# getreu/stringsext

Measured on AMD Instinct MI355X. Metric: GiB/s scanned, higher is better.
Workload: dtype u8

## Files before the change

### stringsext_amd/csrc/sx_api.cpp

```cpp
#include "sx_ctx.hpp"

using namespace sx;

namespace sx {
PinnedPool::Block PinnedPool::take(size_t bytes) {
    {
        std::lock_guard<std::mutex> g(mu);
        size_t best = free_blocks.size();
        for (size_t i = 0; i < free_blocks.size(); i++)
            if (free_blocks[i].cap >= bytes && (best == free_blocks.size() || free_blocks[i].cap < free_blocks[best].cap)) best = i;
        if (best < free_blocks.size() && free_blocks[best].cap <= 4 * bytes + (4u << 20)) {
            Block b = free_blocks[best];
            free_blocks.erase(free_blocks.begin() + (long)best);
            return b;
        }
    }
    Block b;
    const size_t cap = bytes + bytes / 8 + (1u << 20);
    if (hipHostMalloc(&b.p, cap, hipHostMallocNonCoherent) != hipSuccess) { b.p = nullptr; return b; }
    b.cap = cap;
    return b;
}
void PinnedPool::give(Block b) {
    if (!b.p) return;
// ... 254 lines not shown
                         + ", requested=" + std::to_string(hip_device) + "); the scan only runs on the GPU";
        delete ctx;
        return SX_E_NO_DEVICE;
    }
    ctx->device = hip_device;
    auto fail = [&](const char* what, hipError_t err) {
        g_create_error = std::string(what) + ": " + hipGetErrorString(err);
        sx_destroy(ctx);
        return SX_E_HIP;
    };
    if ((e = hipSetDevice(hip_device)) != hipSuccess) return fail("hipSetDevice", e);
    ctx->dev.resize((size_t)n_missions);
    const uint32_t cap = ctx->opt.record_capacity ? ctx->opt.record_capacity : (1u << 20);
    {
        int cus = 0;
        if (hipDeviceGetAttribute(&cus, hipDeviceAttributeMultiprocessorCount, hip_device) == hipSuccess && cus > 0) ctx->n_cus = (unsigned)cus;
        if (ctx->sw.scan_blocks_per_cu >= 0) ctx->scan_blocks_per_cu = (unsigned)ctx->sw.scan_blocks_per_cu;
        if (ctx->sw.region_cap >= 0) ctx->region_cap = (uint32_t)ctx->sw.region_cap;
        if (ctx->sw.scan_cus) ctx->n_cus = (unsigned)ctx->sw.scan_cus;
    }
    int prio_lo = 0, prio_hi = 0;
    (void)hipDeviceGetStreamPriorityRange(&prio_lo, &prio_hi);
    if (ctx->sw.prio_n >= 0) {
        if (ctx->sw.prio_n >= 1) prio_lo = ctx->sw.prio_scan;
        if (ctx->sw.prio_n >= 2) prio_hi = ctx->sw.prio_post;
        fprintf(stderr, "[sx] stream priorities: scan %d, post %d\n", prio_lo, prio_hi);
    }
    const bool per_mission = (ctx->opt.flags & SX_OPT_MISSION_STREAMS) || ctx->sw.mission_streams;
    if ((e = hipStreamCreateWithPriority(&ctx->post_stream, hipStreamNonBlocking, prio_hi)) != hipSuccess) return fail("hipStreamCreate", e);
    if (!per_mission && (e = hipStreamCreateWithPriority(&ctx->scan_stream, hipStreamNonBlocking, prio_lo)) != hipSuccess)
        return fail("hipStreamCreate", e);
// ... 55 lines not shown
            if (d.h_runs) (void)hipHostFree(d.h_runs);
            if (d.ev_runs) (void)hipEventDestroy(d.ev_runs);
            if (d.stream_w) (void)hipStreamDestroy(d.stream_w);
            if (d.h_tot) (void)hipHostFree(d.h_tot);
            if (d.h_small) (void)hipHostFree(d.h_small);
            for (hipEvent_t e : d.wave_ev) if (e) (void)hipEventDestroy(e);
            if (d.stream && d.stream != ctx->scan_stream) (void)hipStreamDestroy(d.stream);
        }
        for (int i = 0; i < 2; i++) {
            if (ctx->ing_pin[i]) (void)hipHostFree(ctx->ing_pin[i]);
            if (ctx->ing_dev[i]) (void)hipFree(ctx->ing_dev[i]);
        }
        if (ctx->copy_stream) (void)hipStreamDestroy(ctx->copy_stream);
        if (ctx->d2h_stream) (void)hipStreamDestroy(ctx->d2h_stream);
        if (ctx->scan_stream) (void)hipStreamDestroy(ctx->scan_stream);
        if (ctx->d_cache) (void)hipFree(ctx->d_cache);
        if (ctx->post_stream) (void)hipStreamDestroy(ctx->post_stream);
        if (ctx->merge_copy_stream) (void)hipStreamDestroy(ctx->merge_copy_stream);
        if (ctx->d_merge) (void)hipFree(ctx->d_merge);
        if (ctx->d_result) (void)hipFree(ctx->d_result);
        if (ctx->d_result_up) (void)hipFree(ctx->d_result_up);
        if (ctx->d_text) (void)hipFree(ctx->d_text);
        if (ctx->d_print_scratch) (void)hipFree(ctx->d_print_scratch);
        if (ctx->d_print_missions) (void)hipFree(ctx->d_print_missions);
        for (uint8_t* p : ctx->d_select) if (p) (void)hipFree(p);
        if (ctx->d_select_scratch) (void)hipFree(ctx->d_select_scratch);
        if (ctx->d_select_scratch2) (void)hipFree(ctx->d_select_scratch2);
        if (ctx->d_distinct) (void)hipFree(ctx->d_distinct);
        for (hipEvent_t e : ctx->merge_ev) if (e) (void)hipEventDestroy(e);
        for (hipEvent_t e : ctx->slab_ev) if (e) (void)hipEventDestroy(e);
// ... 248 lines not shown
```

### stringsext_amd/csrc/sx_ctx.hpp

```cpp
#pragma once
#include <hip/hip_runtime_api.h>
#include <stdio.h>
#include <stdlib.h>
#include <string.h>
#include <errno.h>
#include <fcntl.h>
#include <sys/mman.h>
#include <sys/stat.h>
#include <unistd.h>

#include <algorithm>
#include <atomic>
#include <chrono>
#include <condition_variable>
#include <deque>
#include <functional>
#include <mutex>
#include <string>
#include <thread>
#include <unordered_map>
#include <vector>

#include "sx_host.hpp"
#include "sx_switches.hpp"
#include "sx_stage_b_plan.hpp"

namespace sx {

double now_ms();
constexpr size_t kSmallReadBytes = 4096;
extern double g_tl_t0;
extern int g_tl_on;
#define SX_TL(...) do { if (sx::g_tl_on) { fprintf(stderr, "[tl %+8.3f] ", sx::now_ms() - sx::g_tl_t0); fprintf(stderr, __VA_ARGS__); fputc('\n', stderr); } } while (0)

struct RunList {
    std::vector<sx_run> own;
    const sx_run* p = nullptr;
    size_t n = 0;
    bool on_device = false;
    bool skipped = false;
// ... 97 lines not shown

struct sx_ctx {
    std::shared_ptr<sx::PinnedPool> pool = std::make_shared<sx::PinnedPool>();
    std::shared_ptr<std::atomic<uint64_t>> dev_epoch = std::make_shared<std::atomic<uint64_t>>(0);
    std::vector<sx::Mission> missions;
    std::vector<sx::ScannerState> states;
    std::vector<sx::MissionDev> dev;
    bool host_only = false;
    bool sharded_call = false, single_piece = true;
    int device = -1;
    sx_options opt{};
    sx::Switches sw;
    std::string err;
    sx_stats stats{};
    hipStream_t scan_stream = nullptr, post_stream = nullptr;
    uint8_t* d_cache = nullptr;
    uint64_t d_cache_cap = 0;
    hipStream_t merge_copy_stream = nullptr;
    hipEvent_t merge_ev[3] = { nullptr, nullptr, nullptr };
    hipEvent_t slab_ev[3] = { nullptr, nullptr, nullptr };
    std::atomic<bool> slab_copy_pending{ false };
    uint8_t* d_merge = nullptr; uint64_t d_merge_cap = 0, merge_out_room = 0, merge_n_out = 0;
    uint8_t* d_result = nullptr; uint64_t d_result_cap = 0;
    uint8_t* d_result_up = nullptr; uint64_t d_result_up_cap = 0;
    uint8_t* d_text = nullptr; uint64_t d_text_cap = 0;
    uint8_t* d_print_scratch = nullptr; uint64_t d_print_scratch_cap = 0;
    uint8_t* d_print_missions = nullptr;
    uint8_t* d_select[2] = { nullptr, nullptr }; uint64_t d_select_cap[2] = { 0, 0 };
    std::shared_ptr<std::atomic<uint64_t>> select_epoch[2] = { std::make_shared<std::atomic<uint64_t>>(0), std::make_shared<std::atomic<uint64_t>>(0) };
    uint64_t select_calls = 0;
    uint8_t* d_select_scratch = nullptr; uint64_t d_select_scratch_cap = 0;
    uint8_t* d_select_scratch2 = nullptr; uint64_t d_select_scratch2_cap = 0;
    uint8_t* d_distinct = nullptr; uint64_t d_distinct_cap = 0;
    bool merge_async = false;
    bool merge_copy_pending[2] = { false, false };
    uint64_t merge_parts = 0;
    uint64_t merged_out_bytes = 0;
    double out_density = 0;
    hipEvent_t ev_interleaved = nullptr;
    std::atomic<bool> interleave_pending{ false };
    std::mutex mu;
    std::mutex err_mu;
    std::recursive_mutex grow_mu;
    void set_err(std::string text) { std::lock_guard<std::mutex> g(err_mu); err = std::move(text); }
    unsigned n_cus = 256, scan_blocks_per_cu = 8;
    hipStream_t copy_stream = nullptr;
    hipStream_t d2h_stream = nullptr;
    uint8_t* ing_pin[2] = { nullptr, nullptr };
    uint8_t* ing_dev[2] = { nullptr, nullptr };
    uint64_t ing_cap = 0, ing_dev_cap = 0;
    uint32_t region_cap = 64;
    std::vector<uint32_t> dense;
    uint8_t* d_input = nullptr;
    uint64_t d_input_cap = 0;
    uint64_t ondemand_fetches = 0;
    std::vector<uint64_t> last_runs;
    std::vector<char> wave_pred;
    std::vector<double> wave_density;
    std::vector<char> wave_off;
    std::vector<sx::RunList> shard_runs;
// ... 78 lines not shown
int read_back_sync(sx_ctx* ctx, sx::MissionDev& d, hipStream_t s, void* host_dst, const void* dev_src, size_t bytes);
int read_back_async(sx_ctx* ctx, hipStream_t s, void* pinned_dst, const void* dev_src, size_t bytes);
int ensure_scratch(sx_ctx* ctx, uint64_t bytes);
int ensure_capacity(sx_ctx* ctx, ScanSlot& s, uint32_t cap);
int ensure_rp(sx_ctx* ctx, MissionDev& d, int slot, uint64_t bytes);
int ensure_cache(sx_ctx* ctx, uint64_t bytes);
unsigned usable_cpus();
unsigned replay_threads(const sx_ctx* ctx);
void begin_call(sx_ctx* ctx);
void fill_segment_info(const MissionFindings& s, sx_segment_info* info);

ScanParams scan_params(const sx_ctx* ctx, int mission, const ScanSlot& s, const uint8_t* d_bytes, uint64_t len,
                       uint32_t parity, uint64_t min_chars);
int stage_a_launch(sx_ctx* ctx, const std::vector<int>& which, const uint8_t* d_bytes, uint64_t len,
                   const std::vector<uint32_t>& parity, const std::vector<uint64_t>& min_chars, int si);
struct ReplayJob;
int ensure_copy_stream(sx_ctx* ctx);
bool result_stays_on_device(const sx_ctx* ctx, const ReplayJob& job);
int merge_drain(sx_ctx* ctx);
int slab_copy_drain(sx_ctx* ctx);
int stage_a_finish(sx_ctx* ctx, const std::vector<int>& which, const uint8_t* d_bytes, uint64_t len,
                   const std::vector<uint32_t>& parity, const std::vector<uint64_t>& min_chars, int si,
                   std::vector<RunList>* out, bool cut_into_pieces = false, const ReplayJob* wave_job = nullptr);
int device_runs(sx_ctx* ctx, const std::vector<int>& which, const uint8_t* d_bytes, uint64_t len,
                const std::vector<uint32_t>& parity, const std::vector<uint64_t>& min_chars,
                std::vector<RunList>* out);

struct ReplayJob {
    uint64_t len = 0;
    int file_id = -1;
// ... 97 lines not shown
```

### stringsext_amd/csrc/sx_device.hpp

```cpp
#pragma once
#include <cstdlib>
#include <hip/hip_runtime_api.h>
#include <stdint.h>

#include "../../include/stringsext_amd.h"

namespace sx {

constexpr uint32_t kTileBytes = 1024;

struct DevRun {
    uint64_t start;
    uint32_t len;
    uint32_t chars_flags;
};
constexpr uint32_t kRecStartOpen = 0x80000000u;
constexpr uint32_t kRecEndOpen = 0x40000000u;
constexpr uint32_t kRecCharsMask = 0x3FFFFFFFu;
constexpr uint32_t kRecInvalidLen = 0xFFFFFFFFu, kRecInvalidFlags = 0xFFFFFFFFu;

constexpr uint32_t kStatBase = 32, kStatShards = 16, kStatStride = 32, kCounterWords = kStatBase + kStatShards * kStatStride;

enum ClassifierKind : uint32_t {
    kClsSingleByteLut = 0,
// ... 250 lines not shown
size_t merge_scratch_bytes(uint32_t n);
hipError_t merge_sorted_records(const DevRun* recs, uint32_t n, uint64_t min_chars, void* scratch, size_t scratch_bytes,
                                sx_run* out, uint32_t* out_count, hipStream_t stream);

hipError_t launch_scan(ClassifierKind kind, const ScanParams& p, hipStream_t stream);
constexpr int kFusedMax = 3;
struct FusedParams {
    ScanParams m[kFusedMax];
    const uint8_t* data;
    uint64_t len;
    uint32_t subchunk;
    uint32_t fsh[kFusedMax][4];
    uint32_t cand_f[kFusedMax];
    uint32_t pf_zero[kFusedMax];
};
int fused_slot_of(ClassifierKind kind, const ScanParams& p);
hipError_t launch_scan_fused(const FusedParams& fp, uint32_t used, hipStream_t stream, int prefilter_override);
hipError_t launch_fill_background(uint8_t* dst, uint64_t first_index, uint64_t len, uint64_t seed,
                                  hipStream_t stream);
hipError_t launch_read_sum(const uint8_t* src, uint64_t len, uint64_t* out, hipStream_t stream, uint32_t subchunk = 0, uint32_t rot = 0);
hipError_t launch_gather(const uint8_t* src, uint8_t* dst, const uint64_t* seg_src, const uint64_t* seg_dst,
                         const uint32_t* seg_len, uint32_t n, hipStream_t stream);

}
```

### stringsext_amd/csrc/sx_fused.hip

```cpp
#include "sx_scan_core.hpp"

namespace sx {

struct NoCls {};

SX_DEV u32 shr1_keep(u32 v, u32 old) { return __builtin_amdgcn_update_dpp(old, v, 0x138, 0xF, 0xF, false); }
SX_DEV u32 ror1(u32 v) { return __builtin_amdgcn_mov_dpp(v, 0x13C, 0xF, 0xF, false); }

static_assert(offsetof(FusedParams, m) == 0, "late_params addresses m[slot] from the start of the kernel-argument segment");
typedef const __attribute__((address_space(4))) ScanParams* KArgMission;
SX_DEV KArgMission late_params(u32 slot) {
    asm volatile("" : "+s"(slot));
    return (KArgMission)__builtin_amdgcn_kernarg_segment_ptr() + slot;
}

struct LateEmitter {
    u32 slot, wave;
    u32 rcount, heavy_n;
    SX_DEV void append(bool want, u64 start, u64 end, u32 chars, u32 flags) {
        const u64 m = __ballot(want);
        if (m == 0) return;
        const KArgMission mp = late_params(slot);
        const u32 cap = mp->region_cap;
        DevRun* const recs = mp->recs;
// ... 314 lines not shown
                    const u32 suf = trailing_ones16(S.c.g63 & 0xFFFFu);
                    const u32 s63 = starts_before(*cls, toff, after);
                    os = after - suf;
                    och = (u32)__popc((s63 & 0xFFFFu) >> (16u - suf));
                    ofl = 0;
                }
                S.em.append(lane == 0, os, sub_end, och, ofl | kRecEndOpen);
            }
            S.em.end_region();
        }
    };
    finish(s0); finish(s1); finish(s2);
}

template <class C0, class C1, class C2>
static hipError_t launch_f(const FusedParams& fp, uint32_t used, hipStream_t stream, int prefilter_override) {
    const u64 waves = (fp.len + fp.subchunk - 1) / fp.subchunk;
    const u64 blocks = (waves + 3) / 4;
    if (blocks == 0) return hipSuccess;
    FusedParams q = fp;
    int mode = 1;
    if ((used & 2u) && Prefilter<C1>::mode_for(fp.m[1]) != 1) mode = Prefilter<C1>::mode_for(fp.m[1]);
    if ((used & 4u) && mode && Prefilter<C2>::mode_for(fp.m[2]) != 1) mode = Prefilter<C2>::mode_for(fp.m[2]) == 0 ? 0 : 2;
    if (!(used & 6u)) mode = 0;
    if (prefilter_override == 0) mode = 0; else if (prefilter_override == 2 && mode == 1) mode = 2;
    q.pf_zero[0] = 0; q.pf_zero[1] = Prefilter<C1>::zero_bits(fp.m[1]); q.pf_zero[2] = Prefilter<C2>::zero_bits(fp.m[2]);
    if (mode == 1) hipLaunchKernelGGL((scan_kernel_fused<C0, C1, C2, 1>), dim3((unsigned)blocks), dim3(256), 0, stream, q);
    else if (mode == 2) hipLaunchKernelGGL((scan_kernel_fused<C0, C1, C2, 2>), dim3((unsigned)blocks), dim3(256), 0, stream, q);
    else hipLaunchKernelGGL((scan_kernel_fused<C0, C1, C2, 0>), dim3((unsigned)blocks), dim3(256), 0, stream, q);
    return hipGetLastError();
}

int fused_slot_of(ClassifierKind kind, const ScanParams& p) {
    if (p.region_cap == 0 || p.persistent) return -1;
    if (kind == kClsUtf8Range2) return 0;
    if (kind == kClsUtf16Range) return p.big_endian ? 2 : 1;
    return -1;
}

hipError_t launch_scan_fused(const FusedParams& fp, uint32_t used, hipStream_t stream, int prefilter_override) {
    u32 parity = 0;
    if (used & 2u) parity = fp.m[1].parity & 1u; else if (used & 4u) parity = fp.m[2].parity & 1u;
    FusedParams q = fp;
    for (int s = 0; s < kFusedMax; s++) {
        if (!((used >> s) & 1u)) continue;
        q.data = fp.m[s].data; q.len = fp.m[s].len; q.subchunk = fp.m[s].subchunk;
        const u32 c = std::min<u32>(fp.m[s].cand_bytes, 12u);
        q.cand_f[s] = c;
        u32 have = 1;
        const u32 sh0 = have < c ? 1u : 0u; have += sh0;
        const u32 sh1 = have < c ? std::min(have, c - have) : 0u; have += sh1;
        const u32 rem = c - have;
        const u32 sh2 = std::min(have, rem), sh3 = rem;
        q.fsh[s][0] = sh0; q.fsh[s][1] = sh1; q.fsh[s][2] = sh2; q.fsh[s][3] = sh3;
    }
#define SX_ARG(...) __VA_ARGS__
#define SX_F(U, P, A, B, C) if (used == U && parity == P) return launch_f<A, B, C>(q, used, stream, prefilter_override);
    SX_F(1u, 0u, Utf8Range2, NoCls, NoCls)
    SX_F(7u, 0u, Utf8Range2, SX_ARG(Utf16RangeT<0, 0>), SX_ARG(Utf16RangeT<1, 0>))
    SX_F(7u, 1u, Utf8Range2, SX_ARG(Utf16RangeT<0, 1>), SX_ARG(Utf16RangeT<1, 1>))
    SX_F(3u, 0u, Utf8Range2, SX_ARG(Utf16RangeT<0, 0>), NoCls)
    SX_F(3u, 1u, Utf8Range2, SX_ARG(Utf16RangeT<0, 1>), NoCls)
    SX_F(5u, 0u, Utf8Range2, NoCls, SX_ARG(Utf16RangeT<1, 0>))
    SX_F(5u, 1u, Utf8Range2, NoCls, SX_ARG(Utf16RangeT<1, 1>))
    SX_F(6u, 0u, NoCls, SX_ARG(Utf16RangeT<0, 0>), SX_ARG(Utf16RangeT<1, 0>))
    SX_F(6u, 1u, NoCls, SX_ARG(Utf16RangeT<0, 1>), SX_ARG(Utf16RangeT<1, 1>))
#undef SX_F
#undef SX_ARG
    return hipErrorInvalidValue;
}

}
// ... 1 lines not shown
```

### stringsext_amd/csrc/sx_schedule.cpp

```cpp
#include "sx_ctx.hpp"
#include <thread>

using namespace sx;

namespace sx {

uint64_t piece_bytes(const sx_ctx* ctx, uint64_t len) {
    uint64_t piece = 0;
    bool halves = false;
    if (ctx->sw.piece_mib >= 0) piece = (uint64_t)ctx->sw.piece_mib << 20;
    else if (len >= (16ull << 30) && ctx->missions.size() >= 2 && !(ctx->opt.flags & (SX_OPT_NO_FUSED_SCAN | SX_OPT_MISSION_STREAMS | SX_OPT_RESULT_ON_DEVICE))) {
        piece = ((len / 100) * 50 + kInputBufLen - 1) / kInputBufLen * kInputBufLen;
        halves = true;
    }
    if (piece == 0 || (!halves && len < 2 * piece)) return len;
    for (const Mission& m : ctx->missions) if (m.is_dbcs()) return len;
    return piece / kInputBufLen * kInputBufLen;
}

static uint64_t seq_piece_bytes(const sx_ctx* ctx, uint64_t len) {
    uint64_t piece = 0;
    if (ctx->sw.seq_piece_kib >= 0) {
        piece = (uint64_t)ctx->sw.seq_piece_kib << 10;
        if (piece == 0) return len;
    } else if (ctx->sw.seq_piece_mib >= 0) {
        piece = (uint64_t)ctx->sw.seq_piece_mib << 20;
        if (piece == 0) return len;
    } else {
        if (ctx->opt.flags & SX_OPT_RESULT_ON_DEVICE) return len;
        if (ctx->missions.size() < 2 || ctx->out_density <= 0) return len;
        const double out = ctx->out_density * (double)len;
        if (out < 4.0 * (double)(1ull << 30)) return len;
// ... 23 lines not shown
}
int set_entry_params(sx_ctx* ctx, bool carried_state_is_entry, const uint8_t* host_bytes, const uint8_t* d_bytes, uint64_t len,
                     uint64_t stream_off, std::vector<uint32_t>* parity) {
    parity->clear();
    for (size_t k = 0; k < ctx->missions.size(); k++) {
        uint32_t ep = 0, ep_replay = 0;
        int rc = entry_param(ctx, k, carried_state_is_entry ? &ctx->states[k].decoder : nullptr, host_bytes, d_bytes, len,
                             stream_off, &ep, &ep_replay);
        if (rc != SX_OK) return rc;
        parity->push_back(ep);
        ctx->missions[k].buf_entry_skip = ctx->missions[k].is_dbcs() ? ep_replay : 0u;
    }
    return SX_OK;
}

void mission_order(sx_ctx* ctx, std::vector<int>* out) {
    const size_t nm = ctx->missions.size();
    std::vector<int>& order = *out;
    order.resize(nm);
    for (size_t k = 0; k < nm; k++) order[k] = (int)k;
    if (ctx->last_runs.size() != nm) return;
    std::stable_sort(order.begin(), order.end(), [&](int x, int y) { return ctx->last_runs[(size_t)x] > ctx->last_runs[(size_t)y]; });
    const int mode = ctx->sw.busiest_last;
    if (mode) std::reverse(order.begin(), order.end());
    if (mode == 2 && nm >= 3) std::swap(order[nm - 1], order[nm - 2]);
}

int sync_streams_and_return(sx_ctx* ctx, int rc) {
    ctx->merge_async = false;
    (void)merge_drain(ctx);
    for (auto& d : ctx->dev) { (void)hipStreamSynchronize(d.stream); (void)hipStreamSynchronize(d.stream_b); }
    return rc;
}

struct BufferScan {
    const uint8_t* host_bytes = nullptr;
    const uint8_t* d_bytes = nullptr;
    uint64_t len = 0;
    std::vector<int> order;
    std::vector<uint32_t> parity;
    std::vector<uint64_t> minc;
    int slot = 0;
    std::unique_ptr<SparseDeviceBytes> base_view;
    bool whole = false;
    bool skip_scan(const sx_ctx* ctx, size_t k) const {
        return whole && len >= 2 * kInputBufLen && k < ctx->wave_pred.size() && ctx->wave_pred[k] && ctx->missions[k].wave_ok && !ctx->sw.wave_keep_scan
// ... 136 lines not shown
    }
};

int scan_common(sx_ctx* ctx, const uint8_t* host_bytes, const uint8_t* d_bytes, uint64_t len, int file_id,
                       int is_last, sx_result** out, uint32_t slice_base0, sx_result* append_to) {
    const double t_begin = now_ms();
    g_tl_on = ctx->sw.timeline; g_tl_t0 = t_begin;
    SX_TL("scan_common: %llu bytes", (unsigned long long)len);
    const size_t nm = ctx->missions.size();
    ctx->dev_epoch->fetch_add(1);
    ctx->shard_runs_valid = false;
    std::vector<uint64_t> stream0(nm);
    for (size_t k = 0; k < nm; k++) stream0[k] = ctx->states[k].stream_bytes;
    std::vector<int> order;
    mission_order(ctx, &order);
    const uint64_t seq_piece = ctx->host_only ? len : seq_piece_bytes(ctx, len);
    const bool seq = seq_piece < len;
    const uint64_t piece = seq ? seq_piece : piece_bytes(ctx, len);
    const uint64_t n_pieces = len ? (len + piece - 1) / piece : 1;
    ctx->single_piece = n_pieces == 1 && !append_to;
    const uint64_t merged0 = ctx->merged_out_bytes;
    int entry_rc = SX_OK;
    auto make = [&](uint64_t p) {
        BufferScan b;
        const uint64_t off = p * piece;
        b.host_bytes = host_bytes ? host_bytes + off : nullptr;
        b.d_bytes = d_bytes + off;
        b.len = std::min(piece, len - off);
        b.order = order;
        b.whole = true;
        b.slot = (int)(p & 1);
        for (size_t k = 0; k < nm; k++) {
            uint32_t ep = (uint32_t)((stream0[k] + off) & 1);
            if (ctx->missions[k].is_dbcs()) {
// ... 115 lines not shown
    }
    if (given_runs) {
        ctx->shard_runs.assign(nm, RunList{});
        for (size_t k = 0; k < nm; k++) ctx->shard_runs[k].assign(given_runs[k], given_runs[k] + given_n[k]);
    }
    const void* buf_id = d_bytes ? (const void*)d_bytes : (const void*)host_bytes;
    const bool same_buffer = ctx->shard_runs_valid && ctx->shard_runs_off == buf_off && ctx->shard_runs_len == buf_len && ctx->shard_runs_ptr == buf_id;
    const bool scan_now = !given_runs && !(reuse_runs && same_buffer);
    if (given_runs || scan_now) ctx->shard_runs_valid = false;
    BufferScan b;
    {
        int rc = set_entry_params(ctx, buf_off == 0, host_bytes, d_bytes, buf_len, file_stream_off + buf_off, &b.parity);
        if (rc != SX_OK) return rc;
    }
    if (scan_now) {
        b.host_bytes = host_bytes; b.d_bytes = d_bytes; b.len = buf_len; mission_order(ctx, &b.order); b.slot = 0;
        for (size_t k = 0; k < nm; k++) b.minc.push_back(ctx->missions[k].long_run);
        int rc = b.launch(ctx);
        if (rc == SX_OK) rc = b.fetch_base(ctx);
        if (rc != SX_OK) return sync_streams_and_return(ctx, rc);
    }

    ReplayJob job;
    job.len = buf_len; job.file_id = file_id; job.is_last = false;
    job.hi = own_hi - buf_off;
    job.commit_state = job.hi >= buf_len;
    job.slice_base = (uint32_t)(buf_off / kInputBufLen);
    for (size_t k = 0; k < nm; k++) {
        uint64_t lo = own_lo;
        if (start_at && start_at[k] > lo) lo = start_at[k];
// ... 33 lines not shown
```

### stringsext_amd/csrc/sx_stage_a.cpp

```cpp
#include "sx_ctx.hpp"

using namespace sx;

namespace sx {

static bool large_regions_fit(uint64_t len, uint64_t n_regions, uint32_t cap) {
    const uint64_t slots = n_regions * cap;
    return slots < (1ull << 31) && slots * sizeof(DevRun) <= std::max<uint64_t>(256ull << 20, len / 2);
}

static uint32_t subchunk_bytes(const sx_ctx* ctx) {
    const uint32_t sub = ctx->opt.subchunk_bytes ? ctx->opt.subchunk_bytes : 256u * 1024u;
    return std::max<uint32_t>(kTileBytes, sub / kTileBytes * kTileBytes);
}

static bool fusion_allowed(const sx_ctx* ctx) {
    return !(ctx->opt.flags & (SX_OPT_NO_FUSED_SCAN | SX_OPT_MISSION_STREAMS)) && !ctx->sw.mission_streams && ctx->sw.fused && ctx->sw.scan_warm < 0;
}

ScanParams scan_params(const sx_ctx* ctx, int mission, const ScanSlot& s, const uint8_t* d_bytes, uint64_t len,
                       uint32_t parity, uint64_t min_chars) {
    const Mission& m = ctx->missions[(size_t)mission];
    ScanParams p = m.proto;
    p.data = d_bytes; p.len = len; p.subchunk = subchunk_bytes(ctx); p.parity = parity;
    p.pair_lut = ctx->dev[(size_t)mission].d_pair_lut;
    if (p.gb4) {
        p.gb_ranges = ctx->dev[(size_t)mission].d_table ? ctx->dev[(size_t)mission].d_table + kGbN : nullptr;
        p.ubf = m.c.ubf;
        if (!p.gb_ranges) p.gb4 = 0;
    }
    p.wave_prio = ctx->sw.scan_prio;
    p.min_chars = (uint32_t)std::min<uint64_t>(min_chars, kRecCharsMask);
// ... 8 lines not shown
        }
    }
    p.capacity = s.capacity; p.recs = s.d_recs; p.counters = s.d_counters;
    p.region_cap = s.region_cap; p.region_counts = s.d_cnt; p.grid_flags = s.d_grid;
    unsigned occ = ctx->scan_blocks_per_cu;
    p.persistent = (occ >= 1 && occ < 8) ? occ * ctx->n_cus : 0u;
    return p;
}

int stage_a_launch(sx_ctx* ctx, const std::vector<int>& which, const uint8_t* d_bytes, uint64_t len,
                   const std::vector<uint32_t>& parity, const std::vector<uint64_t>& min_chars, int si) {
    if (len == 0) return SX_OK;
    for (size_t k = 0; k < which.size(); k++) {
        MissionDev& d = ctx->dev[(size_t)which[k]];
        ScanSlot& s = d.slot[si];
        if (s.free_pending) { HIP_TRY(ctx, hipStreamWaitEvent(d.stream, s.ev_free, 0)); s.free_pending = false; }
        {
            const uint32_t sub = subchunk_bytes(ctx);
            const uint64_t n_regions = (len + sub - 1) / sub;
            if (ctx->dense.size() != ctx->missions.size()) ctx->dense.assign(ctx->missions.size(), 0);
            s.region_cap = 0; s.n_regions = n_regions;
            const uint32_t dn = ctx->dense[(size_t)which[k]];
            const uint32_t want_cap = dn > 1 ? dn : (dn == 0 ? ctx->region_cap : 0u);
            if (ctx->region_cap && want_cap &&
                (dn > 1 ? large_regions_fit(len, n_regions, want_cap) : n_regions * want_cap < (1ull << 28))) {
                s.region_cap = want_cap;
                int rc = ensure_capacity(ctx, s, (uint32_t)(n_regions * s.region_cap));
                if (rc != SX_OK && dn > 1) {
                    (void)hipGetLastError();
                    ctx->dense[(size_t)which[k]] = 1;
                    s.region_cap = 0;
                    rc = SX_OK;
                }
                if (rc != SX_OK) return rc;
                if (s.region_cap == 0) goto launch;
                if (s.cnt_cap < n_regions) {
                    if (s.d_cnt) HIP_TRY(ctx, hipFree(s.d_cnt));
                    s.d_cnt = nullptr; s.cnt_cap = 0;
// ... 7 lines not shown
        if (dbcs) {
            const uint32_t sub = subchunk_bytes(ctx);
            const uint64_t n_sub = (len + sub - 1) / sub;
            if (s.grid_cap < n_sub) {
                if (s.d_grid) HIP_TRY(ctx, hipFree(s.d_grid));
                s.d_grid = nullptr; s.grid_cap = 0;
                HIP_TRY(ctx, hipMalloc((void**)&s.d_grid, (n_sub + n_sub / 4 + 64) * 4));
                s.grid_cap = n_sub + n_sub / 4 + 64;
            }
        }
    }
    std::vector<char> fused(which.size(), 0);
    std::vector<ScanParams> params(which.size());
    for (size_t k = 0; k < which.size(); k++)
        params[k] = scan_params(ctx, which[k], ctx->dev[(size_t)which[k]].slot[si], d_bytes, len, parity[k], min_chars[k]);
    if (fusion_allowed(ctx)) {
        FusedParams fp{};
        uint32_t used = 0;
        size_t member[kFusedMax] = { 0, 0, 0 };
        for (size_t k = 0; k < which.size(); k++) {
            if (params[k].persistent) continue;
            const int sl = fused_slot_of(ctx->missions[(size_t)which[k]].kind, params[k]);
            if (sl < 0 || (used >> sl) & 1u) continue;
            if (sl >= 1 && (used & 6u) && ((fp.m[(used & 2u) ? 1 : 2].parity ^ params[k].parity) & 1u)) continue;
            used |= 1u << sl; fp.m[sl] = params[k]; member[sl] = k;
        }
        if (__builtin_popcount(used) >= 2 || used == 1u) {
            hipStream_t st = nullptr;
            for (int sl = 0; sl < kFusedMax; sl++) if ((used >> sl) & 1u) {
                MissionDev& d = ctx->dev[(size_t)which[member[sl]]];
                if (!st) st = d.stream;
                HIP_TRY(ctx, hipMemsetAsync(d.slot[si].d_counters, 0, kCounterWords * sizeof(uint32_t), st));
            }
            for (int sl = 0; sl < kFusedMax; sl++) if ((used >> sl) & 1u) HIP_TRY(ctx, hipEventRecord(ctx->dev[(size_t)which[member[sl]]].slot[si].ev0, st));
            HIP_TRY(ctx, launch_scan_fused(fp, used, st, ctx->sw.fused_prefilter));
            bool first = true;
            for (int sl = 0; sl < kFusedMax; sl++) if ((used >> sl) & 1u) {
                ScanSlot& s = ctx->dev[(size_t)which[member[sl]]].slot[si];
                HIP_TRY(ctx, hipEventRecord(s.ev1, st));
                s.fused = true; s.fused_first = first; first = false;
                fused[member[sl]] = 1;
            }
            ctx->stats.fused_launches++;
        }
    }
    for (size_t k = 0; k < which.size(); k++) {
        if (fused[k]) continue;
        MissionDev& d = ctx->dev[(size_t)which[k]];
        ScanSlot& s = d.slot[si];
        s.fused = false; s.fused_first = false;
        const bool dbcs = ctx->missions[(size_t)which[k]].is_dbcs();
        const ScanParams& p = params[k];
        const uint64_t n_sub = (len + p.subchunk - 1) / p.subchunk;
        for (int w = ctx->sw.scan_warm; w > 0; w--) {
            if (dbcs) HIP_TRY(ctx, hipMemsetAsync(s.d_grid, 0, n_sub * 4, d.stream));
            HIP_TRY(ctx, hipMemsetAsync(s.d_counters, 0, kCounterWords * sizeof(uint32_t), d.stream));
            HIP_TRY(ctx, launch_scan(ctx->missions[(size_t)which[k]].kind, p, d.stream));
        }
        if (dbcs) HIP_TRY(ctx, hipMemsetAsync(s.d_grid, 0, n_sub * 4, d.stream));
        HIP_TRY(ctx, hipMemsetAsync(s.d_counters, 0, kCounterWords * sizeof(uint32_t), d.stream));
        HIP_TRY(ctx, hipEventRecord(s.ev0, d.stream));
        HIP_TRY(ctx, launch_scan(ctx->missions[(size_t)which[k]].kind, p, d.stream));
        HIP_TRY(ctx, hipEventRecord(s.ev1, d.stream));
        if (dbcs) { d.grid_of_scan = s.d_grid; d.grid_sub = p.subchunk; d.grid_data = d_bytes; d.grid_len = len; }
    }
// ... 177 lines not shown
        if (ctx->sw.timing)
            fprintf(stderr, "[sx] mission %d: kernel %.2f ms, %u %s, %s %.2f ms, %s %.2f ms -> %zu runs\n", which[k], ms, nrec,
                    regions ? "records (regions)" : (large_regions ? "record slots (large regions)" : "record slots (pool)"), dev_sorted ? (regions ? "device pack+join" : "device sort+join") : "d2h",
                    tc1 - tc0, dev_sorted ? "d2h runs" : "host join", now_ms() - tc1, rl.size());
        ctx->stats.run_records += rl.size();
        ctx->stats.bytes_scanned += len;
        ctx->stats.heavy_tiles += counters[1];
    }
    ctx->stats.device_ms += now_ms() - t0;
    return SX_OK;
}

int device_runs(sx_ctx* ctx, const std::vector<int>& which, const uint8_t* d_bytes, uint64_t len,
                const std::vector<uint32_t>& parity, const std::vector<uint64_t>& min_chars,
                std::vector<RunList>* out) {
    int rc = stage_a_launch(ctx, which, d_bytes, len, parity, min_chars, 0);
    if (rc != SX_OK) return rc;
    return stage_a_finish(ctx, which, d_bytes, len, parity, min_chars, 0, out);
}


}
```

### stringsext_amd/csrc/sx_switches.cpp

```cpp
#include "sx_switches.hpp"

#include <stdio.h>
#include <stdlib.h>

#include <algorithm>

namespace sx {

static bool present(const char* name) { return getenv(name) != nullptr; }
static bool on_unless_0(const char* name) { const char* e = getenv(name); return !(e && !atoi(e)); }
static bool on_if_nonzero(const char* name) { const char* e = getenv(name); return e && atoi(e); }
static int int_or(const char* name, int unset) { const char* e = getenv(name); return e ? atoi(e) : unset; }
static int64_t i64_or(const char* name, int64_t unset) { const char* e = getenv(name); return e ? (int64_t)atoll(e) : unset; }
static int clamped_or(const char* name, int lo, int hi, int unset) { const char* e = getenv(name); return e ? std::max(lo, std::min(hi, atoi(e))) : unset; }
static uint64_t u64_at_least(const char* name, uint64_t lo, uint64_t unset) { const char* e = getenv(name); return e ? std::max<uint64_t>(lo, (uint64_t)atoll(e)) : unset; }

Switches Switches::from_env() {
    Switches s;
    if (const char* e = getenv("SX_PIN_FLAGS")) s.pin_flags = (int64_t)(unsigned)strtoul(e, nullptr, 0);
    s.small_copy = on_unless_0("SX_SMALL_COPY");
    if (const char* e = getenv("SX_REPLAY_THREADS")) s.replay_threads = (int)std::max(1u, std::min(256u, (unsigned)atoi(e)));
    s.result_on_device = on_if_nonzero("SX_RESULT_ON_DEVICE");
    s.scan_blocks_per_cu = int_or("SX_SCAN_BLOCKS_PER_CU", s.scan_blocks_per_cu);
    if (const char* e = getenv("SX_REGION_CAP")) s.region_cap = (int64_t)(uint32_t)atoi(e);
    s.scan_cus = clamped_or("SX_SCAN_CUS", 1, INT32_MAX, s.scan_cus);
    if (const char* e = getenv("SX_PRIO")) s.prio_n = std::max(0, sscanf(e, "%d,%d", &s.prio_scan, &s.prio_post));
    s.mission_streams = present("SX_MISSION_STREAMS");
    s.scan_prio = (uint32_t)int_or("SX_SCAN_PRIO", (int)s.scan_prio);
    s.fused = on_unless_0("SX_FUSED");
    s.fused_prefilter = int_or("SX_FUSED_PREFILTER", s.fused_prefilter);
    s.scan_warm = clamped_or("SX_SCAN_WARM", 0, INT32_MAX, s.scan_warm);
    s.no_large_regions = present("SX_NO_LARGE_REGIONS");
    s.device_join_min = (uint32_t)int_or("SX_DEVICE_JOIN_MIN", (int)s.device_join_min);
    s.no_pieces = present("SX_NO_PIECES");
    s.probe_rot = (uint32_t)int_or("SX_PROBE_ROT", (int)s.probe_rot);
    s.host_replay = present("SX_HOST_REPLAY");
    s.device_replay = present("SX_DEVICE_REPLAY");
    s.host_stitch = present("SX_HOST_STITCH");
    s.no_replay_skip = present("SX_NO_REPLAY_SKIP");
    s.no_grid_bound = present("SX_NO_GRID_BOUND");
    s.no_replay_cache = present("SX_NO_REPLAY_CACHE");
    s.max_region_windows = (uint32_t)clamped_or("SX_MAX_REGION_WINDOWS", 1, INT32_MAX, (int)s.max_region_windows);
// ... 46 lines not shown
```

### stringsext_amd/csrc/sx_switches.hpp

```cpp
#pragma once
#include <stdint.h>

namespace sx {

struct Switches {
    int64_t pin_flags = -1;
    bool small_copy = true;
    int replay_threads = 0;
    bool result_on_device = false;
    int scan_blocks_per_cu = -1;
    int64_t region_cap = -1;
    int scan_cus = 0;
    int prio_n = -1, prio_scan = 0, prio_post = 0;
    bool mission_streams = false;
    uint32_t scan_prio = 0;
    bool fused = true;
    int fused_prefilter = -1;
    int scan_warm = -1;
    bool no_large_regions = false;
    uint32_t device_join_min = 65536;
    bool no_pieces = false;
    uint32_t probe_rot = 0;
    bool host_replay = false;
    bool device_replay = false;
    bool host_stitch = false;
    bool no_replay_skip = false;
    bool no_grid_bound = false;
    bool no_replay_cache = false;
    uint32_t max_region_windows = 0;
// ... 47 lines not shown
```

Before: 4079.

## Add opt-in CU reservation and LDS slot freeing for fused scan beside stage B

Adds two env-gated mechanisms for the fused scan kernel when it runs alongside stage B. One creates a CU-masked stream that leaves some CUs per XCD free. The other pads dynamic LDS so fewer fused blocks fit per CU, leaving slots for stage-B work. It also moves the piece-splitting and fusion-membership logic into a shared plan header, and piece splitting now keys on the actual fused membership rather than mission count. Slot-free waits now go onto the fused stream. Both new knobs default off, but the piece-size and free-wait changes alter the default path slightly.

```diff
diff --git a/stringsext_amd/csrc/sx_api.cpp b/stringsext_amd/csrc/sx_api.cpp
--- a/stringsext_amd/csrc/sx_api.cpp
+++ b/stringsext_amd/csrc/sx_api.cpp
@@ -292,7 +292,10 @@
     const uint32_t cap = ctx->opt.record_capacity ? ctx->opt.record_capacity : (1u << 20);
     {
         int cus = 0;
-        if (hipDeviceGetAttribute(&cus, hipDeviceAttributeMultiprocessorCount, hip_device) == hipSuccess && cus > 0) ctx->n_cus = (unsigned)cus;
+        if (hipDeviceGetAttribute(&cus, hipDeviceAttributeMultiprocessorCount, hip_device) == hipSuccess && cus > 0) ctx->n_cus = ctx->n_cus_hw = (unsigned)cus;
+        int xcd = 0;
+        if (hipDeviceGetAttribute(&xcd, hipDeviceAttributeNumberOfXccs, hip_device) == hipSuccess && xcd > 0) ctx->n_xcd = (unsigned)xcd;
+        else { (void)hipGetLastError(); ctx->n_xcd = 1; }
         if (ctx->sw.scan_blocks_per_cu >= 0) ctx->scan_blocks_per_cu = (unsigned)ctx->sw.scan_blocks_per_cu;
         if (ctx->sw.region_cap >= 0) ctx->region_cap = (uint32_t)ctx->sw.region_cap;
         if (ctx->sw.scan_cus) ctx->n_cus = (unsigned)ctx->sw.scan_cus;
@@ -378,6 +381,7 @@
         if (ctx->copy_stream) (void)hipStreamDestroy(ctx->copy_stream);
         if (ctx->d2h_stream) (void)hipStreamDestroy(ctx->d2h_stream);
         if (ctx->scan_stream) (void)hipStreamDestroy(ctx->scan_stream);
+        if (ctx->scan_stream_room) { (void)hipStreamSynchronize(ctx->scan_stream_room); (void)hipStreamDestroy(ctx->scan_stream_room); }
         if (ctx->d_cache) (void)hipFree(ctx->d_cache);
         if (ctx->post_stream) (void)hipStreamDestroy(ctx->post_stream);
         if (ctx->merge_copy_stream) (void)hipStreamDestroy(ctx->merge_copy_stream);
diff --git a/stringsext_amd/csrc/sx_ctx.hpp b/stringsext_amd/csrc/sx_ctx.hpp
--- a/stringsext_amd/csrc/sx_ctx.hpp
+++ b/stringsext_amd/csrc/sx_ctx.hpp
@@ -24,6 +24,7 @@
 #include "sx_host.hpp"
 #include "sx_switches.hpp"
 #include "sx_stage_b_plan.hpp"
+#include "sx_schedule_plan.hpp"
 
 namespace sx {
 
@@ -151,6 +152,9 @@
     std::string err;
     sx_stats stats{};
     hipStream_t scan_stream = nullptr, post_stream = nullptr;
+    hipStream_t scan_stream_room = nullptr; bool room_stream_tried = false;
+    hipStream_t fused_stream = nullptr; uint32_t fused_idle_lds = 0;
+    uint32_t lds_per_cu = 0;
     uint8_t* d_cache = nullptr;
     uint64_t d_cache_cap = 0;
     hipStream_t merge_copy_stream = nullptr;
@@ -181,6 +185,7 @@
     std::recursive_mutex grow_mu;
     void set_err(std::string text) { std::lock_guard<std::mutex> g(err_mu); err = std::move(text); }
     unsigned n_cus = 256, scan_blocks_per_cu = 8;
+    unsigned n_cus_hw = 256, n_xcd = 8;
     hipStream_t copy_stream = nullptr;
     hipStream_t d2h_stream = nullptr;
     uint8_t* ing_pin[2] = { nullptr, nullptr };
@@ -289,6 +294,9 @@
                        uint32_t parity, uint64_t min_chars);
 int stage_a_launch(sx_ctx* ctx, const std::vector<int>& which, const uint8_t* d_bytes, uint64_t len,
                    const std::vector<uint32_t>& parity, const std::vector<uint64_t>& min_chars, int si);
+plan::ScheduleFlags schedule_flags(const sx_ctx* ctx);
+plan::ScanTraits expected_scan_traits(const sx_ctx* ctx, size_t k, uint32_t parity);
+int choose_scan_room(sx_ctx* ctx, bool beside_stage_b);
 struct ReplayJob;
 int ensure_copy_stream(sx_ctx* ctx);
 bool result_stays_on_device(const sx_ctx* ctx, const ReplayJob& job);
diff --git a/stringsext_amd/csrc/sx_device.hpp b/stringsext_amd/csrc/sx_device.hpp
--- a/stringsext_amd/csrc/sx_device.hpp
+++ b/stringsext_amd/csrc/sx_device.hpp
@@ -288,8 +288,7 @@
     uint32_t cand_f[kFusedMax];
     uint32_t pf_zero[kFusedMax];
 };
-int fused_slot_of(ClassifierKind kind, const ScanParams& p);
-hipError_t launch_scan_fused(const FusedParams& fp, uint32_t used, hipStream_t stream, int prefilter_override);
+hipError_t launch_scan_fused(const FusedParams& fp, uint32_t used, hipStream_t stream, int prefilter_override, uint32_t idle_lds = 0);
 hipError_t launch_fill_background(uint8_t* dst, uint64_t first_index, uint64_t len, uint64_t seed,
                                   hipStream_t stream);
 hipError_t launch_read_sum(const uint8_t* src, uint64_t len, uint64_t* out, hipStream_t stream, uint32_t subchunk = 0, uint32_t rot = 0);
diff --git a/stringsext_amd/csrc/sx_fused.hip b/stringsext_amd/csrc/sx_fused.hip
--- a/stringsext_amd/csrc/sx_fused.hip
+++ b/stringsext_amd/csrc/sx_fused.hip
@@ -352,7 +352,7 @@
 }
 
 template <class C0, class C1, class C2>
-static hipError_t launch_f(const FusedParams& fp, uint32_t used, hipStream_t stream, int prefilter_override) {
+static hipError_t launch_f(const FusedParams& fp, uint32_t used, hipStream_t stream, int prefilter_override, uint32_t idle_lds) {
     const u64 waves = (fp.len + fp.subchunk - 1) / fp.subchunk;
     const u64 blocks = (waves + 3) / 4;
     if (blocks == 0) return hipSuccess;
@@ -363,20 +363,13 @@
     if (!(used & 6u)) mode = 0;
     if (prefilter_override == 0) mode = 0; else if (prefilter_override == 2 && mode == 1) mode = 2;
     q.pf_zero[0] = 0; q.pf_zero[1] = Prefilter<C1>::zero_bits(fp.m[1]); q.pf_zero[2] = Prefilter<C2>::zero_bits(fp.m[2]);
-    if (mode == 1) hipLaunchKernelGGL((scan_kernel_fused<C0, C1, C2, 1>), dim3((unsigned)blocks), dim3(256), 0, stream, q);
-    else if (mode == 2) hipLaunchKernelGGL((scan_kernel_fused<C0, C1, C2, 2>), dim3((unsigned)blocks), dim3(256), 0, stream, q);
-    else hipLaunchKernelGGL((scan_kernel_fused<C0, C1, C2, 0>), dim3((unsigned)blocks), dim3(256), 0, stream, q);
+    if (mode == 1) hipLaunchKernelGGL((scan_kernel_fused<C0, C1, C2, 1>), dim3((unsigned)blocks), dim3(256), idle_lds, stream, q);
+    else if (mode == 2) hipLaunchKernelGGL((scan_kernel_fused<C0, C1, C2, 2>), dim3((unsigned)blocks), dim3(256), idle_lds, stream, q);
+    else hipLaunchKernelGGL((scan_kernel_fused<C0, C1, C2, 0>), dim3((unsigned)blocks), dim3(256), idle_lds, stream, q);
     return hipGetLastError();
 }
 
-int fused_slot_of(ClassifierKind kind, const ScanParams& p) {
-    if (p.region_cap == 0 || p.persistent) return -1;
-    if (kind == kClsUtf8Range2) return 0;
-    if (kind == kClsUtf16Range) return p.big_endian ? 2 : 1;
-    return -1;
-}
-
-hipError_t launch_scan_fused(const FusedParams& fp, uint32_t used, hipStream_t stream, int prefilter_override) {
+hipError_t launch_scan_fused(const FusedParams& fp, uint32_t used, hipStream_t stream, int prefilter_override, uint32_t idle_lds) {
     u32 parity = 0;
     if (used & 2u) parity = fp.m[1].parity & 1u; else if (used & 4u) parity = fp.m[2].parity & 1u;
     FusedParams q = fp;
@@ -393,7 +386,7 @@
         q.fsh[s][0] = sh0; q.fsh[s][1] = sh1; q.fsh[s][2] = sh2; q.fsh[s][3] = sh3;
     }
 #define SX_ARG(...) __VA_ARGS__
-#define SX_F(U, P, A, B, C) if (used == U && parity == P) return launch_f<A, B, C>(q, used, stream, prefilter_override);
+#define SX_F(U, P, A, B, C) if (used == U && parity == P) return launch_f<A, B, C>(q, used, stream, prefilter_override, idle_lds);
     SX_F(1u, 0u, Utf8Range2, NoCls, NoCls)
     SX_F(7u, 0u, Utf8Range2, SX_ARG(Utf16RangeT<0, 0>), SX_ARG(Utf16RangeT<1, 0>))
     SX_F(7u, 1u, Utf8Range2, SX_ARG(Utf16RangeT<0, 1>), SX_ARG(Utf16RangeT<1, 1>))
diff --git a/stringsext_amd/csrc/sx_schedule.cpp b/stringsext_amd/csrc/sx_schedule.cpp
--- a/stringsext_amd/csrc/sx_schedule.cpp
+++ b/stringsext_amd/csrc/sx_schedule.cpp
@@ -5,17 +5,19 @@
 
 namespace sx {
 
+static_assert(plan::kPieceBufLen == kInputBufLen, "sx_schedule_plan.hpp cuts pieces on the slice grid");
+void mission_order(const sx_ctx* ctx, std::vector<int>* out);
+
 uint64_t piece_bytes(const sx_ctx* ctx, uint64_t len) {
-    uint64_t piece = 0;
-    bool halves = false;
-    if (ctx->sw.piece_mib >= 0) piece = (uint64_t)ctx->sw.piece_mib << 20;
-    else if (len >= (16ull << 30) && ctx->missions.size() >= 2 && !(ctx->opt.flags & (SX_OPT_NO_FUSED_SCAN | SX_OPT_MISSION_STREAMS | SX_OPT_RESULT_ON_DEVICE))) {
-        piece = ((len / 100) * 50 + kInputBufLen - 1) / kInputBufLen * kInputBufLen;
-        halves = true;
-    }
-    if (piece == 0 || (!halves && len < 2 * piece)) return len;
-    for (const Mission& m : ctx->missions) if (m.is_dbcs()) return len;
-    return piece / kInputBufLen * kInputBufLen;
+    std::vector<int> order;
+    mission_order(ctx, &order);
+    std::vector<plan::ScanTraits> ts;
+    for (int k : order) {
+        ts.push_back(expected_scan_traits(ctx, (size_t)k, (uint32_t)(ctx->states[(size_t)k].stream_bytes & 1)));
+        if ((size_t)k < ctx->wave_pred.size() && ctx->wave_pred[(size_t)k] && ctx->missions[(size_t)k].wave_ok && !ctx->sw.wave_keep_scan && ctx->sw.wave_replay != 0)
+            ts.back().no_scan = true;
+    }
+    return plan::piece_bytes(len, schedule_flags(ctx), ts.data(), ts.size(), ctx->sw.piece_mib);
 }
 
 static uint64_t seq_piece_bytes(const sx_ctx* ctx, uint64_t len) {
@@ -69,7 +71,7 @@
     return SX_OK;
 }
 
-void mission_order(sx_ctx* ctx, std::vector<int>* out) {
+void mission_order(const sx_ctx* ctx, std::vector<int>* out) {
     const size_t nm = ctx->missions.size();
     std::vector<int>& order = *out;
     order.resize(nm);
@@ -85,6 +87,7 @@
     ctx->merge_async = false;
     (void)merge_drain(ctx);
     for (auto& d : ctx->dev) { (void)hipStreamSynchronize(d.stream); (void)hipStreamSynchronize(d.stream_b); }
+    if (ctx->scan_stream_room) (void)hipStreamSynchronize(ctx->scan_stream_room);
     return rc;
 }
 
@@ -251,10 +254,12 @@
     for (size_t k = 0; k < nm; k++) stream0[k] = ctx->states[k].stream_bytes;
     std::vector<int> order;
     mission_order(ctx, &order);
+    int rc0 = SX_OK;
     const uint64_t seq_piece = ctx->host_only ? len : seq_piece_bytes(ctx, len);
     const bool seq = seq_piece < len;
     const uint64_t piece = seq ? seq_piece : piece_bytes(ctx, len);
     const uint64_t n_pieces = len ? (len + piece - 1) / piece : 1;
+    if (!ctx->host_only && (rc0 = choose_scan_room(ctx, !seq && n_pieces > 1)) != SX_OK) return rc0;
     ctx->single_piece = n_pieces == 1 && !append_to;
     const uint64_t merged0 = ctx->merged_out_bytes;
     int entry_rc = SX_OK;
@@ -400,6 +405,7 @@
         if (rc != SX_OK) return rc;
     }
     if (scan_now) {
+        { const int rr = choose_scan_room(ctx, false); if (rr != SX_OK) return rr; }
         b.host_bytes = host_bytes; b.d_bytes = d_bytes; b.len = buf_len; mission_order(ctx, &b.order); b.slot = 0;
         for (size_t k = 0; k < nm; k++) b.minc.push_back(ctx->missions[k].long_run);
         int rc = b.launch(ctx);
diff --git a/stringsext_amd/csrc/sx_schedule_plan.hpp b/stringsext_amd/csrc/sx_schedule_plan.hpp
--- /dev/null
+++ b/stringsext_amd/csrc/sx_schedule_plan.hpp
@@ -0,0 +1,97 @@
+#pragma once
+#include <stddef.h>
+#include <stdint.h>
+
+#include <vector>
+
+namespace sx {
+namespace plan {
+
+constexpr uint64_t kPieceBufLen = 4096;
+constexpr int kFusedSlots = 3;
+
+enum FusedFamily : int { kFamOther = 0, kFamUtf8Range2 = 1, kFamUtf16Range = 2 };
+struct ScanTraits {
+    int family = kFamOther;
+    bool big_endian = false;
+    uint32_t parity = 0;
+    uint32_t region_cap = 0;
+    bool persistent = false;
+    bool dbcs = false;
+    bool no_scan = false;
+};
+struct ScheduleFlags {
+    bool no_fused_scan = false;
+    bool mission_streams = false;
+    bool result_on_device = false;
+    bool sw_fused = true;
+    bool scan_warm = false;
+};
+
+inline bool fusion_allowed(const ScheduleFlags& f) { return !f.no_fused_scan && !f.mission_streams && f.sw_fused && !f.scan_warm; }
+
+inline int fused_slot(const ScanTraits& t) {
+    if (t.region_cap == 0 || t.persistent || t.no_scan) return -1;
+    if (t.family == kFamUtf8Range2) return 0;
+    if (t.family == kFamUtf16Range) return t.big_endian ? 2 : 1;
+    return -1;
+}
+
+inline uint32_t fused_members(const ScheduleFlags& f, const ScanTraits* ts, size_t n, size_t member[kFusedSlots]) {
+    for (int s = 0; s < kFusedSlots; s++) member[s] = 0;
+    if (!fusion_allowed(f)) return 0;
+    uint32_t used = 0, par[kFusedSlots] = { 0, 0, 0 };
+    for (size_t k = 0; k < n; k++) {
+        const int sl = fused_slot(ts[k]);
+        if (sl < 0 || (used >> sl) & 1u) continue;
+        if (sl >= 1 && (used & 6u) && ((par[(used & 2u) ? 1 : 2] ^ ts[k].parity) & 1u)) continue;
+        used |= 1u << sl; par[sl] = ts[k].parity; member[sl] = k;
+    }
+    return (__builtin_popcount(used) >= 2 || used == 1u) ? used : 0u;
+}
+
+constexpr uint64_t kPiecesFrom = 16ull << 30;
+constexpr uint64_t kDefaultPieces = 2;
+
+inline uint64_t piece_bytes(uint64_t len, const ScheduleFlags& f, const ScanTraits* ts, size_t n, int64_t piece_mib, uint64_t pieces = kDefaultPieces) {
+    uint64_t piece = 0;
+    bool equal = false;
+    if (piece_mib >= 0) piece = (uint64_t)piece_mib << 20;
+    else if (len >= kPiecesFrom && pieces >= 2 && !f.result_on_device) {
+        size_t member[kFusedSlots];
+        if (__builtin_popcount(fused_members(f, ts, n, member)) >= 2) {
+            piece = ((len + pieces - 1) / pieces + kPieceBufLen - 1) / kPieceBufLen * kPieceBufLen;
+            equal = true;
+        }
+    }
+    if (piece == 0 || (!equal && len < 2 * piece)) return len;
+    for (size_t k = 0; k < n; k++) if (ts[k].dbcs) return len;
+    piece = piece / kPieceBufLen * kPieceBufLen;
+    return piece == 0 || piece >= len ? len : piece;
+}
+
+inline bool scan_cu_mask(unsigned n_cus, unsigned n_xcd, unsigned r, int layout, std::vector<uint32_t>* words) {
+    words->clear();
+    if (n_cus == 0 || n_xcd == 0 || n_cus % n_xcd != 0 || (layout != 0 && layout != 1)) return false;
+    const unsigned per = n_cus / n_xcd;
+    if (r >= per) return false;
+    words->assign((n_cus + 31) / 32, 0u);
+    for (unsigned i = 0; i < n_cus; i++) {
+        const unsigned cu = layout == 0 ? i / n_xcd : i % per;
+        if (cu < per - r) (*words)[i / 32] |= 1u << (i % 32);
+    }
+    return true;
+}
+
+constexpr unsigned kScanBlocksPerCu = 8;
+inline uint32_t free_slot_lds_bytes(uint64_t lds_per_cu, unsigned s, uint64_t granule) {
+    if (s < 1 || s > 2 || granule == 0) return 0;
+    const uint64_t fit = kScanBlocksPerCu - s;
+    const uint64_t size = lds_per_cu / fit / granule * granule;
+    if (size == 0 || size > 0xFFFFFFFFull || !(fit * size <= lds_per_cu && lds_per_cu < (fit + 1) * size)) return 0;
+    return (uint32_t)size;
+}
+inline uint64_t lds_granule(uint64_t lds_per_cu) { return lds_per_cu == (160ull << 10) ? 1280 : 512; }
+
+}
+}
diff --git a/stringsext_amd/csrc/sx_stage_a.cpp b/stringsext_amd/csrc/sx_stage_a.cpp
--- a/stringsext_amd/csrc/sx_stage_a.cpp
+++ b/stringsext_amd/csrc/sx_stage_a.cpp
@@ -1,6 +1,8 @@
 #include "sx_ctx.hpp"
 
 using namespace sx;
+
+static_assert(plan::kFusedSlots == kFusedMax, "sx_schedule_plan.hpp deals the fused kernel's slots");
 
 namespace sx {
 
@@ -14,8 +16,65 @@
     return std::max<uint32_t>(kTileBytes, sub / kTileBytes * kTileBytes);
 }
 
-static bool fusion_allowed(const sx_ctx* ctx) {
-    return !(ctx->opt.flags & (SX_OPT_NO_FUSED_SCAN | SX_OPT_MISSION_STREAMS)) && !ctx->sw.mission_streams && ctx->sw.fused && ctx->sw.scan_warm < 0;
+plan::ScheduleFlags schedule_flags(const sx_ctx* ctx) {
+    plan::ScheduleFlags f;
+    f.no_fused_scan = (ctx->opt.flags & SX_OPT_NO_FUSED_SCAN) != 0;
+    f.mission_streams = (ctx->opt.flags & SX_OPT_MISSION_STREAMS) != 0 || ctx->sw.mission_streams;
+    f.result_on_device = (ctx->opt.flags & SX_OPT_RESULT_ON_DEVICE) != 0;
+    f.sw_fused = ctx->sw.fused;
+    f.scan_warm = ctx->sw.scan_warm >= 0;
+    return f;
+}
+plan::ScanTraits scan_traits(const sx_ctx* ctx, int mission, const ScanParams& p) {
+    const Mission& m = ctx->missions[(size_t)mission];
+    plan::ScanTraits t;
+    t.family = m.kind == kClsUtf8Range2 ? plan::kFamUtf8Range2 : (m.kind == kClsUtf16Range ? plan::kFamUtf16Range : plan::kFamOther);
+    t.big_endian = p.big_endian != 0; t.parity = p.parity; t.region_cap = p.region_cap; t.persistent = p.persistent != 0;
+    t.dbcs = m.is_dbcs(); t.no_scan = m.host_sequential();
+    return t;
+}
+static uint32_t wanted_region_cap(const sx_ctx* ctx, size_t k) {
+    const uint32_t dn = k < ctx->dense.size() ? ctx->dense[k] : 0u;
+    return dn > 1 ? dn : (dn == 0 ? ctx->region_cap : 0u);
+}
+plan::ScanTraits expected_scan_traits(const sx_ctx* ctx, size_t k, uint32_t parity) {
+    ScanParams p = ctx->missions[k].proto;
+    p.parity = parity; p.region_cap = ctx->region_cap ? wanted_region_cap(ctx, k) : 0u;
+    p.persistent = (ctx->scan_blocks_per_cu >= 1 && ctx->scan_blocks_per_cu < 8) ? 1u : 0u;
+    return scan_traits(ctx, (int)k, p);
+}
+
+int choose_scan_room(sx_ctx* ctx, bool beside_stage_b) {
+    ctx->fused_stream = nullptr; ctx->fused_idle_lds = 0;
+    if (!beside_stage_b || ctx->host_only || !ctx->scan_stream) return SX_OK;
+    const unsigned r = ctx->sw.scan_reserve_cus, s = ctx->sw.scan_free_slots;
+    if (r && !ctx->room_stream_tried) {
+        ctx->room_stream_tried = true;
+        std::vector<uint32_t> words;
+        const char* why = nullptr;
+        if (!plan::scan_cu_mask(ctx->n_cus_hw, ctx->n_xcd, r, ctx->sw.scan_reserve_layout, &words)) why = "no CU would be left to the scan";
+        else if (hipExtStreamCreateWithCUMask(&ctx->scan_stream_room, (uint32_t)words.size(), words.data()) != hipSuccess) {
+            (void)hipGetLastError();
+            ctx->scan_stream_room = nullptr;
+            why = "hipExtStreamCreateWithCUMask failed";
+        }
+        if (ctx->sw.timing) {
+            if (why) fprintf(stderr, "[sx] SX_SCAN_RESERVE_CUS=%u: %s (%u CUs, %u XCDs): the plain scan stream\n", r, why, ctx->n_cus_hw, ctx->n_xcd);
+            else fprintf(stderr, "[sx] SX_SCAN_RESERVE_CUS=%u: fused launches beside stage B go to a stream of %u - %u CUs (layout %d)\n", r, ctx->n_cus_hw, r * ctx->n_xcd, ctx->sw.scan_reserve_layout);
+        }
+    }
+    if (r) ctx->fused_stream = ctx->scan_stream_room;
+    if (s) {
+        if (!ctx->lds_per_cu) {
+            int v = 0;
+            if (hipDeviceGetAttribute(&v, hipDeviceAttributeMaxSharedMemoryPerMultiprocessor, ctx->device) != hipSuccess || v <= 0) { (void)hipGetLastError(); v = 64 << 10; }
+            ctx->lds_per_cu = (uint32_t)v;
+            if (ctx->sw.timing) fprintf(stderr, "[sx] SX_SCAN_FREE_SLOTS=%u: %u bytes of LDS per CU, %u idle bytes per fused block\n", s, ctx->lds_per_cu,
+                                        plan::free_slot_lds_bytes(ctx->lds_per_cu, s, plan::lds_granule(ctx->lds_per_cu)));
+        }
+        ctx->fused_idle_lds = plan::free_slot_lds_bytes(ctx->lds_per_cu, s, plan::lds_granule(ctx->lds_per_cu));
+    }
+    return SX_OK;
 }
 
 ScanParams scan_params(const sx_ctx* ctx, int mission, const ScanSlot& s, const uint8_t* d_bytes, uint64_t len,
@@ -54,14 +113,13 @@
     for (size_t k = 0; k < which.size(); k++) {
         MissionDev& d = ctx->dev[(size_t)which[k]];
         ScanSlot& s = d.slot[si];
-        if (s.free_pending) { HIP_TRY(ctx, hipStreamWaitEvent(d.stream, s.ev_free, 0)); s.free_pending = false; }
         {
             const uint32_t sub = subchunk_bytes(ctx);
             const uint64_t n_regions = (len + sub - 1) / sub;
             if (ctx->dense.size() != ctx->missions.size()) ctx->dense.assign(ctx->missions.size(), 0);
             s.region_cap = 0; s.n_regions = n_regions;
             const uint32_t dn = ctx->dense[(size_t)which[k]];
-            const uint32_t want_cap = dn > 1 ? dn : (dn == 0 ? ctx->region_cap : 0u);
+            const uint32_t want_cap = wanted_region_cap(ctx, (size_t)which[k]);
             if (ctx->region_cap && want_cap &&
                 (dn > 1 ? large_regions_fit(len, n_regions, want_cap) : n_regions * want_cap < (1ull << 28))) {
                 s.region_cap = want_cap;
@@ -99,26 +157,28 @@
     std::vector<ScanParams> params(which.size());
     for (size_t k = 0; k < which.size(); k++)
         params[k] = scan_params(ctx, which[k], ctx->dev[(size_t)which[k]].slot[si], d_bytes, len, parity[k], min_chars[k]);
-    if (fusion_allowed(ctx)) {
+    auto wait_free = [&](ScanSlot& s, hipStream_t st) -> hipError_t {
+        if (!s.free_pending) return hipSuccess;
+        s.free_pending = false;
+        return hipStreamWaitEvent(st, s.ev_free, 0);
+    };
+    {
         FusedParams fp{};
-        uint32_t used = 0;
         size_t member[kFusedMax] = { 0, 0, 0 };
-        for (size_t k = 0; k < which.size(); k++) {
-            if (params[k].persistent) continue;
-            const int sl = fused_slot_of(ctx->missions[(size_t)which[k]].kind, params[k]);
-            if (sl < 0 || (used >> sl) & 1u) continue;
-            if (sl >= 1 && (used & 6u) && ((fp.m[(used & 2u) ? 1 : 2].parity ^ params[k].parity) & 1u)) continue;
-            used |= 1u << sl; fp.m[sl] = params[k]; member[sl] = k;
-        }
-        if (__builtin_popcount(used) >= 2 || used == 1u) {
-            hipStream_t st = nullptr;
+        std::vector<plan::ScanTraits> traits(which.size());
+        for (size_t k = 0; k < which.size(); k++) traits[k] = scan_traits(ctx, which[k], params[k]);
+        const uint32_t used = plan::fused_members(schedule_flags(ctx), traits.data(), traits.size(), member);
+        for (int sl = 0; sl < kFusedMax; sl++) if ((used >> sl) & 1u) fp.m[sl] = params[member[sl]];
+        if (used) {
+            hipStream_t st = ctx->fused_stream;
             for (int sl = 0; sl < kFusedMax; sl++) if ((used >> sl) & 1u) {
                 MissionDev& d = ctx->dev[(size_t)which[member[sl]]];
                 if (!st) st = d.stream;
+                HIP_TRY(ctx, wait_free(d.slot[si], st));
                 HIP_TRY(ctx, hipMemsetAsync(d.slot[si].d_counters, 0, kCounterWords * sizeof(uint32_t), st));
             }
             for (int sl = 0; sl < kFusedMax; sl++) if ((used >> sl) & 1u) HIP_TRY(ctx, hipEventRecord(ctx->dev[(size_t)which[member[sl]]].slot[si].ev0, st));
-            HIP_TRY(ctx, launch_scan_fused(fp, used, st, ctx->sw.fused_prefilter));
+            HIP_TRY(ctx, launch_scan_fused(fp, used, st, ctx->sw.fused_prefilter, ctx->fused_idle_lds));
             bool first = true;
             for (int sl = 0; sl < kFusedMax; sl++) if ((used >> sl) & 1u) {
                 ScanSlot& s = ctx->dev[(size_t)which[member[sl]]].slot[si];
@@ -134,6 +194,7 @@
         MissionDev& d = ctx->dev[(size_t)which[k]];
         ScanSlot& s = d.slot[si];
         s.fused = false; s.fused_first = false;
+        HIP_TRY(ctx, wait_free(s, d.stream));
         const bool dbcs = ctx->missions[(size_t)which[k]].is_dbcs();
         const ScanParams& p = params[k];
         const uint64_t n_sub = (len + p.subchunk - 1) / p.subchunk;
@@ -341,7 +402,8 @@
 int device_runs(sx_ctx* ctx, const std::vector<int>& which, const uint8_t* d_bytes, uint64_t len,
                 const std::vector<uint32_t>& parity, const std::vector<uint64_t>& min_chars,
                 std::vector<RunList>* out) {
-    int rc = stage_a_launch(ctx, which, d_bytes, len, parity, min_chars, 0);
+    int rc = choose_scan_room(ctx, true);
+    if (rc == SX_OK) rc = stage_a_launch(ctx, which, d_bytes, len, parity, min_chars, 0);
     if (rc != SX_OK) return rc;
     return stage_a_finish(ctx, which, d_bytes, len, parity, min_chars, 0, out);
 }
diff --git a/stringsext_amd/csrc/sx_switches.cpp b/stringsext_amd/csrc/sx_switches.cpp
--- a/stringsext_amd/csrc/sx_switches.cpp
+++ b/stringsext_amd/csrc/sx_switches.cpp
@@ -26,6 +26,9 @@
     s.scan_cus = clamped_or("SX_SCAN_CUS", 1, INT32_MAX, s.scan_cus);
     if (const char* e = getenv("SX_PRIO")) s.prio_n = std::max(0, sscanf(e, "%d,%d", &s.prio_scan, &s.prio_post));
     s.mission_streams = present("SX_MISSION_STREAMS");
+    s.scan_reserve_cus = (unsigned)clamped_or("SX_SCAN_RESERVE_CUS", 0, 255, (int)s.scan_reserve_cus);
+    s.scan_reserve_layout = clamped_or("SX_SCAN_RESERVE_LAYOUT", 0, 1, s.scan_reserve_layout);
+    s.scan_free_slots = (unsigned)clamped_or("SX_SCAN_FREE_SLOTS", 0, 2, (int)s.scan_free_slots);
     s.scan_prio = (uint32_t)int_or("SX_SCAN_PRIO", (int)s.scan_prio);
     s.fused = on_unless_0("SX_FUSED");
     s.fused_prefilter = int_or("SX_FUSED_PREFILTER", s.fused_prefilter);
diff --git a/stringsext_amd/csrc/sx_switches.hpp b/stringsext_amd/csrc/sx_switches.hpp
--- a/stringsext_amd/csrc/sx_switches.hpp
+++ b/stringsext_amd/csrc/sx_switches.hpp
@@ -13,6 +13,9 @@
     int scan_cus = 0;
     int prio_n = -1, prio_scan = 0, prio_post = 0;
     bool mission_streams = false;
+    unsigned scan_reserve_cus = 0;
+    int scan_reserve_layout = 0;
+    unsigned scan_free_slots = 0;
     uint32_t scan_prio = 0;
     bool fused = true;
     int fused_prefilter = -1;
```

After: 4076 (median of 2 runs). No clear change (-0.1%).
